# LTLA/batchelor

Hardware: AMD Instinct MI355X
Metric: cells/sec corrected (reducedMNN engine, 50 PCs) (higher is better)
Workload: dtype fp16 MFMA candidate pass (f32 accumulate) + FP64 exact re-rank; 1 GPU; config3: 8 synthetic Gaussian batches x 100000 cells x 50 PCs, k=20, merge.order=1..8, inputs resident in HBM; parallelism=single GPU, exact_fallback_queries=990

## Files before the change

batchelor_amd/csrc/abi.hip:

```cpp
#include <algorithm>
#include <chrono>
#include <climits>
#include <cstddef>
#include <cmath>
#include <cstdlib>
#include <cstring>
#include <functional>
#include <limits>
#include <memory>
#include <thread>
#include <vector>

#include "bmx_common.hpp"
#include "bmx_ops.hpp"
#include "engine.hpp"
#include "gene_var_host.hpp"
#include "host_xfer.hpp"
#include "mnn_correct.hpp"
#include "rccl_dyn.hpp"
#include "resident_batches.hpp"

struct bmx_engine {
    std::unique_ptr<bmx::Engine> impl;
};
// ... 141 lines not shown
        }
    });
}

void bmx_trim_caches(void) {
    bmx::DevBlockCache::release_global();
    bmx::StreamPool::release_all();
}

int64_t bmx_last_knn_exact_fallbacks(void) { return g_last_fallbacks; }

void bmx_set_force_exact_knn(int32_t on) { g_force_exact = on; }

int32_t bmx_dev_set(const char* name, int32_t value) {
    if (!name) return BMX_ERR_ARG;
    bmx::DevKnobs& k = bmx::dev_knobs();
    const std::string n(name);
    if (n == "knn_tier") k.knn_tier = value;
    else if (n == "sample") k.sample = value;
    else if (n == "split_c") k.split_c = value;
    else if (n == "force_c") k.force_c = value;
    else if (n == "no_margin") k.no_margin = value;
    else if (n == "asv_fast") k.asv_fast = value;
    else if (n == "asv_cap") k.asv_cap = value;
    else if (n == "sample_split") k.sample_split = value;
    else if (n == "lk_seed") k.lk_seed = value;
    else if (n == "asv_modes") k.asv_modes = value;
    else if (n == "asv_sync") k.asv_sync = value;
    else if (n == "tau_replay") k.tau_replay = value;
    else if (n == "exchange_always") k.exchange_always = value;
    else if (n == "refine_wave") k.refine_wave = value;
    else if (n == "asv_wide") k.asv_wide = value;
    else if (n == "asv_chunk") k.asv_chunk = value;
    else if (n == "reset") k = bmx::DevKnobs();
    else {
        g_last_error = "bmx_dev_set: unknown knob '" + n + "'";
        return BMX_ERR_ARG;
    }
    return BMX_OK;
}

int32_t bmx_dev_get(const char* name, int64_t* value) {
    if (!name || !value) return BMX_ERR_ARG;
    return guarded([&] {
        const std::string n(name);
        unsigned long long t[8];
        if (n == "asv_literal_cells" || n == "asv_fallback_cells" || n == "asv_tiled_cells") {
            bmx::asv_tally_read(t, false);
            *value = (int64_t)t[n == "asv_literal_cells" ? 0 : (n == "asv_fallback_cells" ? 1 : 2)];
        } else if (n == "asv_ticks_stream" || n == "asv_ticks_wait" || n == "asv_ticks_cells") {
            bmx::asv_ticks_read(t);
            *value = (int64_t)t[n == "asv_ticks_stream" ? 0 : (n == "asv_ticks_wait" ? 1 : 2)];
        } else if (n == "asv_ticks_literal" || n == "asv_ticks_chains" || n == "asv_literal_addends" || n == "asv_chain_tiles") {
            bmx::asv_ticks_read(t);
            *value = (int64_t)t[n == "asv_ticks_literal" ? 4 : (n == "asv_ticks_chains" ? 5 : (n == "asv_literal_addends" ? 6 : 7))];
        } else if (n == "delta_gene_tile" || n == "delta_pair_chunk") {
            *value = n == "delta_gene_tile" ? bmx::DELTA_GENE_TILE : bmx::DELTA_PAIR_CHUNK;
        } else if (n == "delta_sparse_gene_tile") {
            *value = bmx::DELTA_SPARSE_GENE_TILE;
        } else if (n == "genevar_gene_tile" || n == "genevar_chunk") {
            *value = n == "genevar_gene_tile" ? bmx::GENEVAR_GENE_TILE : bmx::GENEVAR_CHUNK;
        } else if (n == "cluster_sparse_gene_tile") {
            *value = bmx::CLUSTER_SPARSE_GENE_TILE;
        } else if (n == "pca_sparse_row_segment") {
            *value = bmx::PCA_SPARSE_ROW_SEGMENT;
        } else if (n == "asv_tally_reset") {
// ... 747 lines not shown
```

batchelor_amd/csrc/host_basics.hpp:

```cpp
#pragma once
#include <cstdint>
#include <stdexcept>
#include <string>

#include "../../include/batchelor_mi355x.h"

namespace bmx {

struct Error : std::runtime_error {
    int code;
    Error(int c, const std::string& m) : std::runtime_error(m), code(c) {}
};

struct DevKnobs {
    int knn_tier = 0;
    int sample = -1;
    int split_c = 0;
    int force_c = 0;
    int no_margin = 0;
    int asv_fast = 0;
    int asv_cap = -1;
    int asv_modes = 0;
    int asv_sync = 0;
    int tau_replay = 0;
    int lk_seed = 1;
    int sample_split = -1;
    int exchange_always = 0;
    int refine_wave = 0;
    int asv_wide = 0;
    int asv_chunk = 0;
};

inline int cdiv(int64_t a, int64_t b) { return (int)((a + b - 1) / b); }
inline int64_t round_up(int64_t a, int64_t b) { return (a + b - 1) / b * b; }

}
```

batchelor_amd/csrc/knn.hip:

```cpp
#include "knn_internal.hpp"

#include <algorithm>
#include <atomic>
#include <chrono>
#include <cmath>
#include <cstdio>
#include <thread>

namespace bmx {
namespace {

using namespace sel;

__global__ void colsum_partial(const double* __restrict__ X, const int32_t* __restrict__ rows, int n, int d,
                               int rows_per_block, int stride, double* __restrict__ partial) {
    __shared__ double sm[4][64];
    const int c0 = threadIdx.x & 63, rl = threadIdx.x >> 6;
    const int r0 = blockIdx.x * rows_per_block;
    const int r1 = min(n, r0 + rows_per_block);
    for (int cb = 0; cb < d; cb += 64) {
        const int c = cb + c0;
        double s = 0.0;
        if (c < d)
            for (int r = r0 + rl; r < r1; r += 4) {
// ... 83 lines not shown
        pe.eps_qr = 6.0;
        pe.eps_split = 1.5 * 3.03 * 2.0 * 1.52587890625e-05;
        pe.eps_den = 0.0;
        pe.scaled = 0;
    }
    return pe;
}

}

int candidate_tiers(int d, int k, int nr, Tier out[2]) {
    const int only = dev_knobs().knn_tier;
    int n = 0;
    if (k > 36) return 0;
    const int KS1 = k <= 20 ? BMX_KS1 : 48, KS2 = k <= 20 ? 24 : 40;
    const int ns1 = f16_pick_ns(d, KS1);
    if (ns1 && nr > 2 * KS1 && (only == 0 || only == 1)) out[n++] = Tier{1, ns1, KS1};
    const int ns2 = bf16_pick_ns(d);
    if (ns2 && !(KS2 == 40 && ns2 > 16) && nr > 2 * KS2 && (only == 0 || only == 2)) out[n++] = Tier{2, ns2, KS2};
    return n;
}

namespace {

void candidate_pass(hipStream_t stream, KnnWorkspace& ws, const Tier& T, const double* X, const int32_t* ref_rows, int nr,
                    const double* Qs, const int32_t* qrs, int nq, int d, int k, int32_t* io, double* dout,
                    int32_t* flagged, double* flag_bound, const float* seed_d2, const double* centre, double* kth_out) {
    const int NS = T.NS, KS = T.KS;
    ws.last_variant = T.id == 1 ? 3 : 2;
    const PassPlan plan = plan_candidate_pass(T.id, NS, KS, T.id == 1 ? 256 : 32 * bf16_ncons(NS, KS),
                                              T.id == 1 ? f16_rows_per_slot(NS, KS) : 32, nq, nr, seed_d2 != nullptr, dev_knobs());
    const int nq_pad = plan.nq_pad, nqb = plan.nqb, S = plan.S, C = plan.C, chunk_len = plan.chunk_len, nr_pad = plan.nr_pad;
    const int nchunks = C;
    if (debug_prints())
        fprintf(stderr, "[bmx] knn tier %d: nq=%d nr=%d d=%d NS=%d KS=%d S=%d C=%d chunk=%d full-range blocks=%d of %d\n", T.id,
                nq, nr, d, NS, KS, S, C, chunk_len, C > 1 ? plan.n_full : nqb, nqb);

    const int KPw = 8 * NS;
    float* pq = ws.pq.reserve((size_t)nq_pad * KPw);
    float* pr = ws.pr.reserve((size_t)(nr_pad + 256) * KPw);
    double* qn2 = ws.qn2.reserve(nq_pad);
    double* rn2 = ws.rn2.reserve(nr_pad);
    double* mean = ws.mean.reserve((size_t)d + 2);
    unsigned long long* maxbits = reinterpret_cast<unsigned long long*>(mean + d);
    int32_t* cand = ws.cand.reserve((size_t)nq_pad * nchunks * KS);
    float* cand_v = ws.cand_v.reserve((size_t)nq_pad * nchunks * KS);
    float* tau = ws.tau.reserve((size_t)nq_pad * nchunks);
    uint32_t* tau_g = ws.tau_g.reserve(nq_pad);
    unsigned long long* slots = ws.maxslots.reserve(64 * 16);

    if (!centre) {
        const int cstride = std::max(1, nr / 16384);
        const int ncs = cdiv(nr, cstride);
        const int rpb = 256;
        const int nb = cdiv(ncs, rpb);
        double* red = ws.red.reserve((size_t)nb * d);
        hipLaunchKernelGGL(colsum_partial, dim3(nb), dim3(256), 0, stream, X, ref_rows, ncs, d, rpb, cstride, red);
        BMX_LAUNCH_CHECK();
        hipLaunchKernelGGL(colsum_final, dim3(cdiv(d, 64)), dim3(64), 0, stream, red, nb, d, 1.0 / ncs, mean);
        BMX_LAUNCH_CHECK();
        centre = mean;
    }
    const PassEps pe = tier_pass_eps(T, d);
    PassLaunch L{reinterpret_cast<const uint16_t*>(pq), reinterpret_cast<const uint16_t*>(pr), nqb, 0, plan.sample_range_len,
                 plan.sample_nranges, S, 0, nchunks, tau_g, 1, cand, cand_v, tau};
    const bool no_margin = dev_knobs().no_margin != 0;
    auto go = [&](const PassLaunch& l) {
        return T.id == 1 ? f16_launch(stream, ws, NS, KS, l) : bf16_launch(stream, ws, NS, KS, l);
    };
    bool ok = true;
    unsigned long long* zero_slots = nullptr;
    if (T.id == 1) {
        if (!ws.slots_clean) BMX_HIP(hipMemsetAsync(slots, 0, 64 * 16 * sizeof(unsigned long long), stream));
        float* margin = no_margin ? nullptr : ws.margin.reserve(nq_pad);
        uint32_t* tau_seed = seed_d2 ? ws.tau_seed.reserve(nq_pad) : nullptr;
        f16_prep_all(stream, X, ref_rows, nr, nr_pad, Qs, qrs, nq, nq_pad, d, NS, centre, reinterpret_cast<uint16_t*>(pr),
                     reinterpret_cast<uint16_t*>(pq), rn2, qn2, maxbits, slots, flagged, margin, pe, seed_d2, tau_seed,
                     S == 0 || plan.CS > 1 ? tau_g : nullptr);
        if (margin) {
            L.margin = margin;
            L.k = k;
        }
        L.tau_seed = tau_seed;
        zero_slots = slots;
        ws.slots_clean = false;
        if (S > 0) {
            float* lists = nullptr;
            if (L.nranges > 1 && margin) {
                lists = ws.samp_lists.reserve((size_t)nq_pad * L.nranges * KS);
                L.cand_v = lists;
            }
            ok = go(L);
            if (lists) f16_sample_merge(stream, lists, L.nranges, KS, nq, k, margin, tau_g);
            L.cand_v = cand_v;
        }
    } else {
        ws.slots_clean = false;
        BMX_HIP(hipMemsetAsync(maxbits, 0, sizeof(unsigned long long), stream));
        bf16_prep(stream, X, ref_rows, nr, nr_pad, d, NS, centre, 0, reinterpret_cast<uint16_t*>(pr), rn2, maxbits, slots);
        bf16_prep(stream, Qs, qrs, nq, nq_pad, d, NS, centre, 1, reinterpret_cast<uint16_t*>(pq), qn2, maxbits, slots);
        if (S == 0) {
            hipLaunchKernelGGL(fill_u32, dim3(cdiv(nq_pad, 256)), dim3(256), 0, stream, tau_g, nq_pad, 0xFF800000u);
            BMX_LAUNCH_CHECK();
        }
        if (S > 0) ok = go(L);
        if (seed_d2) {
            hipLaunchKernelGGL(seed_tau_kernel, dim3(cdiv(nq_pad, 256)), dim3(256), 0, stream, seed_d2, qn2, maxbits, nq, nq_pad,
                               pe, tau_g);
            BMX_LAUNCH_CHECK();
        }
        BMX_HIP(hipMemsetAsync(flagged, 0, sizeof(int32_t), stream));
    }
    L.first_begin = 0;
    L.range_len = chunk_len;
    L.nranges = C;
    L.n_full = C > 1 ? plan.n_full : 0;
    L.r_limit = nr_pad;
    L.sample = 0;
    const int replay = T.id == 1 ? dev_knobs().tau_replay : 0;
    if (replay == 2 && ws.replay_idx < ws.tau_rec.size() && ws.tau_rec[ws.replay_idx].cap >= (size_t)nq_pad) {
        hipLaunchKernelGGL(tau_apply_kernel, dim3(cdiv(nq_pad, 256)), dim3(256), 0, stream,
                           (const uint32_t*)ws.tau_rec[ws.replay_idx].p, nq_pad, tau_g);
        BMX_LAUNCH_CHECK();
    }
    ok = ok && go(L);
    if (replay == 1) {
        if (ws.tau_rec.size() <= ws.replay_idx) ws.tau_rec.resize(ws.replay_idx + 1);
        hipLaunchKernelGGL(tau_record_kernel, dim3(cdiv(nq_pad, 256)), dim3(256), 0, stream, (const float*)tau, nchunks, nq_pad,
                           ws.tau_rec[ws.replay_idx].reserve((size_t)nq_pad));
        BMX_LAUNCH_CHECK();
    }
    if (replay) ++ws.replay_idx;
    if (!ok) throw Error(BMX_ERR_ARG, "kNN: unsupported padded dimension");
    refine_launch(stream, ws, plan, KS, pe, PassLists{cand, cand_v, tau, qn2, maxbits}, X, ref_rows, Qs, qrs, nq, d, k, seed_d2,
                  io, dout, flagged, flag_bound, zero_slots, kth_out);
    if (zero_slots) ws.slots_clean = true;
    if (debug_prints()) {
        std::vector<int32_t> hc((size_t)nq * nchunks * KS);
        BMX_HIP(hipMemcpyAsync(hc.data(), cand, hc.size() * sizeof(int32_t), hipMemcpyDeviceToHost, stream));
        ws.sync(stream);
        size_t valid = 0;
        for (int32_t v : hc) valid += v >= 0;
        fprintf(stderr, "[bmx] candidates per query after the top-k pass: %.1f (of %d slots)\n", (double)valid / nq,
                nchunks * KS);
    }
// ... 109 lines not shown
```

batchelor_amd/csrc/knn_f16.hip:

```cpp
#include "knn_internal.hpp"

#include <cmath>
#include <string>

namespace bmx {
namespace {

using namespace sel;
typedef _Float16 f16x8 __attribute__((ext_vector_type(8)));

constexpr int NCONS = 8;
constexpr int NPROD = 2;
#ifndef BMX_NSERV
#define BMX_NSERV 4
#endif
__host__ __device__ constexpr int serv_waves(int NS) { return NS <= 5 ? BMX_NSERV : 2; }
constexpr int NQ = NCONS * 32;
constexpr int QCAP = 64;
#ifndef BMX_DRAIN_MIN
#define BMX_DRAIN_MIN 16
#endif
#ifndef BMX_SPRIO
#define BMX_SPRIO 0
#endif
#ifndef BMX_CPRIO_LO
#define BMX_CPRIO_LO 0
#endif
#ifndef BMX_CPRIO_HI
#define BMX_CPRIO_HI 1
#endif
#ifndef BMX_HEAD
#define BMX_HEAD 4
#endif
#ifndef BMX_RING_MAX
#define BMX_RING_MAX 4
#endif
#ifndef BMX_NPIV
#define BMX_NPIV 4
#endif
#ifndef BMX_PSLEEP
#define BMX_PSLEEP 1
#endif
constexpr int EPI_CONS = 20;
constexpr int DRAIN_MIN = BMX_DRAIN_MIN;
constexpr int HEAD = BMX_HEAD;

__device__ __forceinline__ uint16_t f32_to_f16_bits(float f) {
    const _Float16 h = (_Float16)f;
    return __builtin_bit_cast(uint16_t, h);
}
__device__ __forceinline__ float f16_bits_to_f32(uint16_t b) { return (float)__builtin_bit_cast(_Float16, b); }

__host__ __device__ __forceinline__ double f16_scale(double max_n2) {
    const double rm = sqrt(max_n2);
    if (!(rm > 1e-150) || !(rm < 1e150)) return 1.0;
    int e = 0;
    (void)frexp(48.0 / rm, &e);
    return ldexp(1.0, e - 1);
}

template <int PHASE>
__device__ __forceinline__ double prep_rows(char* smem_pp, int block, const double* __restrict__ X,
                                            const int32_t* __restrict__ rows, int n, int d, int NS,
                                            const double* __restrict__ mean, int is_query, uint16_t* __restrict__ P,
                                            double* __restrict__ n2, unsigned long long* __restrict__ max_slots,
                                            double scale) {
    const int K = 16 * NS;
    float* xs = reinterpret_cast<float*>(smem_pp);
// ... 125 lines not shown
        double m = __longlong_as_double((long long)slots[(size_t)threadIdx.x * 16]);
        for (int o = 1; o < 64; o <<= 1) m = fmax(m, __shfl_xor(m, o));
        if (threadIdx.x == 0) {
            sh_max = m;
            if (blockIdx.x == 0) {
                *max_n2_bits = (unsigned long long)__double_as_longlong(m);
                if (flagged0) *flagged0 = 0;
            }
        }
    }
    __syncthreads();
    const double max_rn2 = sh_max;
    const double scale = f16_scale(max_rn2);
    if ((int)blockIdx.x < nrb) {
        (void)prep_rows<1>(smem_pp, blockIdx.x, X, rrows, nr, d, NS, mean, 0, Pr, rn2, nullptr, scale);
        return;
    }
    const int qb = blockIdx.x - nrb;
    const double s = prep_rows<1>(smem_pp, qb, Q, qrows, nq, d, NS, mean, 1, Pq, qn2, nullptr, scale);
    const int rr = threadIdx.x >> 3, sub = threadIdx.x & 7;
    if (sub == 0) {
        const int q = qb * 32 + rr;
        const bool live = q < nq;
        const double nn = live ? qn2[q] : 0.0;
        (void)s;
        if (margin) margin[q] = live ? pass_margin(nn, max_rn2, pe) : 0.f;
        uint32_t ts = 0xFF800000u;
        if (seed_d2) ts = live ? pass_seed_tau((double)seed_d2[q], nn, max_rn2, pe) : f32_orderable(-__builtin_inff());
        if (tau_seed) tau_seed[q] = ts;
        if (tau_init) tau_init[q] = ts;
    }
}

__host__ __device__ constexpr int lds_fixed_bytes() { return NCONS * QCAP * 20 + NQ * 4 + NQ * 4 + NQ * 4 + 512; }
__host__ __device__ constexpr int ring_slots_for(int NS, int LCAP, int TP) {
    const int rest = 160 * 1024 - lds_fixed_bytes() - NQ * LCAP * 8;
    const int n = rest / (TP * 2 * NS * 1024);
    return n > BMX_RING_MAX ? BMX_RING_MAX : n;
}
#ifndef BMX_LCAP_MAX
#define BMX_LCAP_MAX 56
#endif
#ifndef BMX_TP_MAX
#define BMX_TP_MAX 2
#endif
__host__ __device__ constexpr int tile_pairs_for(int NS, int KS) {
    return (BMX_TP_MAX >= 2 && KS + 16 <= BMX_LCAP_MAX && ring_slots_for(NS, KS + 16, 2) >= 3) ? 2 : 1;
}
__host__ __device__ constexpr int list_cap(int NS, int KS) {
    const int TP = tile_pairs_for(NS, KS);
    for (int c = BMX_LCAP_MAX; c >= KS + 16; c -= 8)
        if (ring_slots_for(NS, c, TP) >= (TP == 2 ? 3 : 2)) return c;
    return KS + 16 <= 64 ? KS + 16 : 64;
}

__device__ __forceinline__ int lds_load_volatile(const int* p) {
    return __hip_atomic_load(p, __ATOMIC_RELAXED, __HIP_MEMORY_SCOPE_WORKGROUP);
}
__device__ __forceinline__ int mbcnt64(unsigned long long m) {
    return __builtin_amdgcn_mbcnt_hi((uint32_t)(m >> 32), __builtin_amdgcn_mbcnt_lo((uint32_t)m, 0u));
}

#ifdef BMX_STAMPS
__device__ unsigned long long bmx_dbg16[48];
#define STAMP() __builtin_readcyclecounter()
#endif

template <int NS, int KS, int LCAP, bool SAMPLE>
__global__ __launch_bounds__((NCONS + NPROD + serv_waves(NS)) * 64) void knn_topk_f16(
    const uint16_t* __restrict__ Pq, const uint16_t* __restrict__ PrF, int first_begin, int range_len, int r_limit,
    int n_full, int nranges, int out_chunk0, int out_nchunks, uint32_t* __restrict__ tau_g, int32_t* __restrict__ cand,
    float* __restrict__ cand_v, float* __restrict__ tau_out, const float* __restrict__ margin_g, int kq,
    const uint32_t* __restrict__ tau_seed) {
    constexpr int TILE_BYTES = NS * 1024;
    constexpr int TP = tile_pairs_for(NS, KS);
    constexpr int SLOT_BYTES = TP * 2 * TILE_BYTES;
    constexpr int NSLOT = ring_slots_for(NS, LCAP, TP);
    static_assert(NSLOT >= 2, "LDS ring");
    static_assert(LCAP <= 64 && LCAP > KS, "one list entry per lane during compaction");
    constexpr int KEEP_MAX = KS + 11 < LCAP - 4 ? KS + 11 : LCAP - 4;
    static_assert(KEEP_MAX >= KS, "list capacity");
    constexpr int NSERV = serv_waves(NS);
    static_assert(NCONS % NSERV == 0 && (NCONS / NSERV) % 2 == 0, "a service wave's consumers: whole groups of 64 queries");
    static_assert((QCAP & (QCAP - 1)) == 0 && QCAP >= 64, "queue positions wrap by masking; one group can hold 64 records");

    extern __shared__ __attribute__((aligned(16))) char smem[];
    char* ring = smem;
    unsigned long long* lists = reinterpret_cast<unsigned long long*>(smem + NSLOT * SLOT_BYTES);
    float* qvals = reinterpret_cast<float*>(lists + NQ * LCAP);
    uint32_t* qtags = reinterpret_cast<uint32_t*>(qvals + NCONS * QCAP * 4);
    int* cnt = reinterpret_cast<int*>(qtags + NCONS * QCAP);
    float* tauL = reinterpret_cast<float*>(cnt + NQ);
    float* mgL = tauL + NQ;
    int* ready = reinterpret_cast<int*>(mgL + NQ);
    int* done = ready + NSLOT;
    int* wrL = done + NSLOT;
    int* rdL = wrL + NCONS;
    int* stL = rdL + NCONS;
#ifdef BMX_EXP_ROWFILTER
    float* rtau = reinterpret_cast<float*>(stL + NCONS);
    if (threadIdx.x < 32) rtau[threadIdx.x] = -__builtin_inff();
#endif

    const int tid = threadIdx.x, lane = tid & 63;
    const int wave = __builtin_amdgcn_readfirstlane(tid >> 6);
    int qblock = blockIdx.x, rng = 0, nrng = 1, r_begin = first_begin, r_end = r_limit;
    if ((int)blockIdx.x >= n_full) {
        const int nsplit = (gridDim.x - n_full) / nranges, jx = blockIdx.x - n_full;
        rng = jx / nsplit;
        qblock = n_full + (jx - rng * nsplit);
        nrng = nranges;
        r_begin = first_begin + rng * range_len;
        r_end = min(r_limit, r_begin + range_len);
    }
    const int ntiles = (r_end - r_begin) >> 5;
    const int nslots = ntiles / (2 * TP);
    const int out_chunk = out_chunk0 + rng;
    if (tid < 2 * NSLOT + 3 * NCONS) ready[tid] = 0;
    if (tid < NQ) {
        cnt[tid] = 0;
        tauL[tid] = (!SAMPLE && tau_g) ? orderable_f32(tau_g[qblock * NQ + tid]) : __builtin_inff();
        mgL[tid] = (!SAMPLE && margin_g) ? margin_g[qblock * NQ + tid] : 0.f;
    }
    __syncthreads();
    const bool shared_tau = !SAMPLE && tau_g != nullptr && nrng > 1;

#ifdef BMX_STAMPS
    unsigned long long dbg_ncomp = 0, dbg_comp = 0, dbg_rounds = 0;
#endif
    auto compact = [&](const int c, const int jj, const bool exact) __attribute__((always_inline)) {
        unsigned long long* mylists = lists + c * 32 * LCAP;
        int* mycnt = cnt + c * 32;
        const int n_raw = __builtin_amdgcn_readfirstlane(lds_load_volatile(&mycnt[jj]));
        const int n = n_raw < LCAP ? n_raw : LCAP;
        if (n <= KS && (n < kq || margin_g == nullptr)) return;
#ifdef BMX_STAMPS
        const unsigned long long c0 = STAMP();
        ++dbg_ncomp;
#endif
        const unsigned long long raw = lane < n ? mylists[jj * LCAP + lane] : 0ull;
        const uint32_t key =
            lane < n ? (((f32_orderable(__uint_as_float((uint32_t)(raw >> 32))) >> 1) & ~63u) | (uint32_t)lane)
                     : 0x7FFFFFFFu;
        unsigned long long M = 0, keep = 0;
        int pl = 0, kept = 0x7FFFFFFF, nkeep = 0;
        uint32_t pk = 0;
        float newtau = 0.f;
        bool cut_done = false;
        auto select_rank = [&](unsigned long long B, const int target) __attribute__((always_inline)) {
            int it = 0;
            for (;;) {
                const int rot = (it * 29 + jj * 7) & 63;
// ... 495 lines not shown
                    for (int u = 0; u < 4; ++u) {
                        unsigned long long mu = __builtin_amdgcn_ballot_w64(g[u] < tau);
                        if (mu == 0) continue;
                        const int c = __builtin_popcountll(mu);
                        if (wr + c - rd_seen > QCAP) {
                            wait_room(c);
                            const float tl =
                                __hip_atomic_load(&tauL[wave * 32 + j], __ATOMIC_RELAXED, __HIP_MEMORY_SCOPE_WORKGROUP);
                            tau = tl < tau ? tl : tau;
                            mu = __builtin_amdgcn_ballot_w64(g[u] < tau);
                        }
                        if (mu) {
                            spill(u, mu);
                            __atomic_signal_fence(__ATOMIC_SEQ_CST);
                            lane0_store(&wrL[wave], wr);
                        }
                    }
#ifdef BMX_STAMPS
                    dbg_evc += STAMP() - dbg_e0;
#endif
                    return mn;
                }
                wait_room(tot);
            }
#pragma unroll
            for (int u = 0; u < 4; ++u) spill(u, m[u]);
#ifdef BMX_STAMPS
            dbg_evc += STAMP() - dbg_e0;
#endif
            return mn;
        }
    };

    if (wave >= NCONS / 2)
        __builtin_amdgcn_s_setprio(BMX_CPRIO_HI);
    else
        __builtin_amdgcn_s_setprio(BMX_CPRIO_LO);
    __builtin_amdgcn_s_waitcnt(0x0F70);
    if (nslots > 0) {
        typedef __attribute__((address_space(3))) const char* lds_cptr;
        typedef __attribute__((address_space(3))) const f32x4* lds_f4ptr;
        lds_cptr ring_lane = (lds_cptr)ring + lane * 16;
        asm volatile("" : "+v"(ring_lane));
        spin_until_staged(0, 0);
        __atomic_signal_fence(__ATOMIC_SEQ_CST);
        {
            const lds_f4ptr tp = (lds_f4ptr)ring_lane;
#pragma unroll
            for (int s = 0; s < NS; ++s) {
                a[s] = tp[s * 64];
                b[s] = tp[(NS + s) * 64];
            }
        }
        if constexpr (TP == 1) hand_back(0);
        poll(1 % NSLOT);
        auto tile_pair = [&](const lds_f4ptr tp, const int t0, const int hand_back_pos) __attribute__((always_inline)) {
            f32x16 accA, accB;
#ifdef BMX_EXP_ROWFILTER
            if constexpr (!SAMPLE) {
#ifdef BMX_EXP_ROWFILTER_NOLDS
#pragma unroll
                for (int u = 0; u < 4; ++u) {
                    rt[u] = f32x4{rt0, rt0, rt0, rt0};
                    asm volatile("" : "+v"(rt[u]));
                }
#else
// ... 19 lines not shown
                __builtin_amdgcn_sched_group_barrier(0x008, 1, 0);
                __builtin_amdgcn_sched_group_barrier(0x100, 1, 0);
            }
            __builtin_amdgcn_sched_barrier(0);
            if (hand_back_pos >= 0) hand_back(hand_back_pos);
            const float mnA = sift(accA, t0);
            const float mnB = sift(accB, t0 + 1);
            if constexpr (SAMPLE) {
                sample_insert(fminf(fminf(mnA, mnB), mnB));
            }
        };
        for (int sl0 = 0; sl0 < nslots; sl0 += NSLOT) {
#pragma unroll
            for (int k = 0; k < NSLOT; ++k) {
                const int sl = sl0 + k;
                if (sl >= nslots) break;
                const int kn = (k + 1) % NSLOT;
                if constexpr (TP == 2) {
                    __builtin_amdgcn_s_waitcnt(0xC07F);
                    tile_pair((lds_f4ptr)(ring_lane + k * SLOT_BYTES + 2 * TILE_BYTES), 4 * sl, k);
                }
                __builtin_amdgcn_s_waitcnt(0xC07F);
                if constexpr (!SAMPLE) asm("v_min_f32 %0, %0, %1" : "+v"(tau) : "v"(tau_next));
                spin_until_staged(sl + 1, kn);
                __atomic_signal_fence(__ATOMIC_SEQ_CST);
                poll((kn + 1) % NSLOT);
                tile_pair((lds_f4ptr)(ring_lane + kn * SLOT_BYTES), 2 * TP * sl + 2 * (TP - 1), TP == 1 ? kn : -1);
            }
        }
    }
    __builtin_amdgcn_s_setprio(0);

    if constexpr (SAMPLE) {
        const uint32_t mine = f32_orderable(best[KS / 2 - 1]), other = __shfl_xor(mine, 32);
        uint32_t start = max(mine, other);
        if constexpr (KS / 2 <= 24) {
            if (margin_g && kq >= 1 && kq <= KS) {
                float part[KS / 2];
#pragma unroll
                for (int e = 0; e < KS / 2; ++e) part[e] = __shfl_xor(best[e], 32);
                float uk = __builtin_inff();
#pragma unroll
                for (int i = 0; i < KS / 2; ++i) {
                    int r = i;
#pragma unroll
                    for (int e = 0; e < KS / 2; ++e) r += (part[e] < best[i] || (part[e] == best[i] && h == 1)) ? 1 : 0;
                    uk = r == kq - 1 ? best[i] : uk;
                }
                uk = fminf(uk, __shfl_xor(uk, 32));
                const float tm = uk + margin_g[q] + fabsf(uk) * 2.384185791015625e-07f;
                if (tm == tm) start = min(start, f32_orderable(tm));
            }
        }
        if (h == 0) {
            if (nrng > 1) atomicMin(&tau_g[q], start);
            else tau_g[q] = tau_seed ? min(start, tau_seed[q]) : start;
        }
        if (nrng > 1 && cand_v) {
            float* dst = cand_v + ((int64_t)q * nrng + rng) * KS + h * (KS / 2);
#pragma unroll
            for (int e = 0; e < KS / 2; e += 4)
                *reinterpret_cast<f32x4*>(dst + e) = f32x4{best[e], best[e + 1], best[e + 2], best[e + 3]};
        }
#ifdef BMX_STAMPS
        if (lane == 0) {
            atomicAdd(&bmx_dbg16[0], STAMP() - dbg_t0);
            atomicAdd(&bmx_dbg16[1], dbg_spin);
            atomicAdd(&bmx_dbg16[8], (unsigned long long)ntiles);
            atomicAdd(&bmx_dbg16[9], 1ull);
        }
#endif
    } else {
        __atomic_signal_fence(__ATOMIC_SEQ_CST);
        lane0_store(&wrL[wave], wr);
        lane0_store(&stL[wave], 2);
        while (__builtin_amdgcn_readfirstlane(lds_load_volatile(&stL[wave])) != 3) __builtin_amdgcn_s_sleep(2);
        __atomic_signal_fence(__ATOMIC_SEQ_CST);
        out_lists(wave, 0, EPI_CONS);
#ifdef BMX_STAMPS
        if (lane == 0) {
            atomicAdd(&bmx_dbg16[0], STAMP() - dbg_t0);
            atomicAdd(&bmx_dbg16[1], dbg_spin);
            atomicAdd(&bmx_dbg16[6], dbg_evt);
            atomicAdd(&bmx_dbg16[7], dbg_grp);
            atomicAdd(&bmx_dbg16[8], (unsigned long long)ntiles);
            atomicAdd(&bmx_dbg16[9], 1ull);
            atomicAdd(&bmx_dbg16[10], dbg_evc);
            atomicAdd(&bmx_dbg16[12], dbg_qwait);
        }
#endif
    }
}

template <int NS, int KS>
void launch(hipStream_t stream, KnnWorkspace& ws, const PassLaunch& L) {
    constexpr int LCAP = list_cap(NS, KS);
    constexpr int TP = tile_pairs_for(NS, KS);
    constexpr size_t lds =
        (size_t)ring_slots_for(NS, LCAP, TP) * TP * 2 * NS * 1024 + (size_t)NQ * LCAP * 8 + lds_fixed_bytes();
    static_assert(lds <= 160 * 1024, "LDS budget");
    ensure_dynamic_lds(reinterpret_cast<const void*>(&knn_topk_f16<NS, KS, LCAP, false>), lds);
    ensure_dynamic_lds(reinterpret_cast<const void*>(&knn_topk_f16<NS, KS, LCAP, true>), lds);
    std::pair<hipEvent_t, hipEvent_t> ev{nullptr, nullptr};
    if (ws.profile) {
        ev = ws.next_events(L.sample ? 0 : 1);
        BMX_HIP(hipEventRecord(ev.first, stream));
    }
    if (!L.sample)
        ws.last_kernel = "knn_topk_f16<" + std::to_string(NS) + ", " + std::to_string(KS) + ", " + std::to_string(LCAP) +
                         ", false>";
    const int items = L.n_full + (L.nqb - L.n_full) * L.nranges;
    if (L.sample)
        hipLaunchKernelGGL((knn_topk_f16<NS, KS, LCAP, true>), dim3(items), dim3((NCONS + NPROD + serv_waves(NS)) * 64), lds, stream,
                           L.pq, L.pr, L.first_begin, L.range_len, L.r_limit, L.n_full, L.nranges, L.out_chunk0,
                           L.out_nchunks, L.tau_g, L.cand, L.cand_v, L.tau, L.margin, L.k, L.tau_seed);
    else
        hipLaunchKernelGGL((knn_topk_f16<NS, KS, LCAP, false>), dim3(items), dim3((NCONS + NPROD + serv_waves(NS)) * 64), lds, stream,
                           L.pq, L.pr, L.first_begin, L.range_len, L.r_limit, L.n_full, L.nranges, L.out_chunk0,
                           L.out_nchunks, L.tau_g, L.cand, L.cand_v, L.tau, L.margin, L.k, (const uint32_t*)nullptr);
    BMX_LAUNCH_CHECK();
    if (ws.profile) BMX_HIP(hipEventRecord(ev.second, stream));
#ifdef BMX_STAMPS
    {
        if (L.sample) fprintf(stderr, "(sample pass) ");
        unsigned long long hh[48];
        BMX_HIP(hipStreamSynchronize(stream));
        BMX_HIP(hipMemcpyFromSymbol(hh, HIP_SYMBOL(bmx_dbg16), sizeof(hh)));
        const double nt = (double)hh[8];
        const double sw = hh[14] ? (double)hh[14] : 1.0;
        fprintf(stderr,
                "[stamps f16] consumers=%.0f tiles/wave=%.0f cyc/tile=%.0f spin/tile=%.0f evpath/tile=%.0f qwait/tile=%.0f "
                "event tiles=%.3f groups/tile=%.3f | service waves=%.0f cyc=%.0f drain=%.0f (%.0f passes, %.0f cyc each) "
                "compact=%.0f (%.0f calls, %.1f rounds each) idle polls=%.0f\n",
                (double)hh[9], nt / hh[9], hh[0] / nt, hh[1] / nt, hh[10] / nt, hh[12] / nt, hh[6] / nt, hh[7] / nt,
                (double)hh[14], hh[13] / sw, hh[2] / sw, hh[3] / sw, hh[3] ? (double)hh[2] / hh[3] : 0.0, hh[5] / sw,
                hh[4] / sw, hh[4] ? (double)hh[11] / hh[4] : 0.0, hh[15] / sw);
        unsigned long long z[48] = {0};
        BMX_HIP(hipMemcpyToSymbol(HIP_SYMBOL(bmx_dbg16), z, sizeof(z)));
    }
#endif
}

}

namespace {
// ... 50 lines not shown
    hipLaunchKernelGGL(knn_prep_f16_rq, dim3(nr_pad / 32 + nq_pad / 32), dim3(256), lds, stream, X, rrows, nr, nr_pad / 32, Q, qrows,
                       nq, d, NS, mean, Pr, Pq, rn2, qn2, (const unsigned long long*)slots, maxbits, flagged0, margin, pe, seed_d2,
                       tau_seed, tau_init);
    BMX_LAUNCH_CHECK();
}

bool f16_launch(hipStream_t stream, KnnWorkspace& ws, int NS, int KS, const PassLaunch& L) {
#define BMX_CASE(N)                       \
    case N:                               \
        if (KS == BMX_KS1)                \
            launch<N, BMX_KS1>(stream, ws, L); \
        else if constexpr (N <= 4)        \
            launch<N, 48>(stream, ws, L); \
        else                              \
            return false;                 \
        return true;
    switch (NS) {
        BMX_CASE(1)
        BMX_CASE(2)
        BMX_CASE(3)
        BMX_CASE(4)
        BMX_CASE(5)
        BMX_CASE(6)
        BMX_CASE(7)
        BMX_CASE(8)
        default:
            return false;
    }
#undef BMX_CASE
}

double f16_scale_host(double max_n2) { return f16_scale(max_n2); }
int f16_rows_per_slot(int NS, int KS) { return 64 * tile_pairs_for(NS, KS); }

}
```

batchelor_amd/csrc/knn_internal.hpp:

```cpp
#pragma once
#include "bmx_common.hpp"
#include "knn_plan.hpp"
#include "knn_select.hpp"

namespace bmx {

struct PassLaunch {
    const uint16_t* pq;
    const uint16_t* pr;
    int nqb, first_begin, range_len, nranges, r_limit, out_chunk0, out_nchunks;
    uint32_t* tau_g;
    int sample;
    int32_t* cand;
    float* cand_v;
    float* tau;
    int n_full = 0;
    const float* margin = nullptr;
    int k = 0;
    const uint32_t* tau_seed = nullptr;
};
int bf16_pick_ns(int d);
int bf16_ncons(int NS, int KS);
void bf16_prep(hipStream_t stream, const double* X, const int32_t* rows, int n, int n_pad, int d, int NS,
               const double* mean, int is_query, uint16_t* P, double* n2, unsigned long long* maxbits,
               unsigned long long* slots);
bool bf16_launch(hipStream_t stream, KnnWorkspace& ws, int NS, int KS, const PassLaunch& L);
int f16_pick_ns(int d, int KS);
int f16_rows_per_slot(int NS, int KS);
void f16_prep_all(hipStream_t stream, const double* X, const int32_t* rrows, int nr, int nr_pad, const double* Q,
                  const int32_t* qrows, int nq, int nq_pad, int d, int NS, const double* mean, uint16_t* Pr, uint16_t* Pq,
                  double* rn2, double* qn2, unsigned long long* maxbits, unsigned long long* slots, int32_t* flagged0,
                  float* margin, const sel::PassEps& pe, const float* seed_d2, uint32_t* tau_seed, uint32_t* tau_init);
bool f16_launch(hipStream_t stream, KnnWorkspace& ws, int NS, int KS, const PassLaunch& L);
void f16_sample_merge(hipStream_t stream, const float* lists, int nranges, int KS, int nq, int k, const float* margin,
                      uint32_t* tau_g);

struct Tier {
    int id;
    int NS, KS;
};
int candidate_tiers(int d, int k, int nr, Tier out[2]);
void search_tiers(hipStream_t stream, KnnWorkspace& ws, const Tier* tiers, int ntiers, int t, const double* X,
                  const int32_t* ref_rows, int nr, const double* Qs, const int32_t* qrs, int nq, int d, int k, int32_t* io,
                  double* dout, const float* seed_d2 = nullptr, const double* centre = nullptr, double* kth_out = nullptr);
int read_count(hipStream_t stream, KnnWorkspace& ws, const int32_t* dev);

struct PassLists {
    const int32_t* cand;
    const float* cand_v;
    const float* tau;
    const double* qn2;
    const unsigned long long* maxbits;
};
void refine_launch(hipStream_t stream, KnnWorkspace& ws, const PassPlan& plan, int KS, const sel::PassEps& pe,
                   const PassLists& lists, const double* X, const int32_t* ref_rows, const double* Qs, const int32_t* qrs,
                   int nq, int d, int k, const float* seed_d2, int32_t* io, double* dout, int32_t* flagged,
                   double* flag_bound, unsigned long long* zero_slots, double* kth_out);

int32_t* launch_bounded_sweep(hipStream_t stream, KnnWorkspace& ws, const double* X, const int32_t* ref_rows, int nr,
                              const double* Qs, const int32_t* qrs, int d, int k, int32_t* io, double* dout,
                              const int32_t* list, const double* bounds, int count, int dev_cap, bool seeded, int32_t* opt);
// ... 13 lines not shown
```

Measured before the change: 9.417 million cells/s.

## Add 64-query-per-wave consumers for the f16 sample pass

Adds a sample-pass kernel variant for the NS=4, KS=32 instance in which each consumer wave handles 64 queries: it issues two MFMAs per loaded reference fragment, keeps per-lane minima directly in registers, and drops the service waves and LDS candidate lists. This raises reuse of each staged reference tile and removes queue and service overhead in the sampling stage. The sample launch is replanned with a doubled query block, so the query-side buffers are padded to the larger size. Because the fragment-min insertion differs from the service-wave path, the sampled thresholds may be looser, which could increase work in later passes. The new path is on by default through a knob.

```diff
diff --git a/batchelor_amd/csrc/abi.hip b/batchelor_amd/csrc/abi.hip
--- a/batchelor_amd/csrc/abi.hip
+++ b/batchelor_amd/csrc/abi.hip
@@ -197,6 +197,7 @@
     else if (n == "refine_wave") k.refine_wave = value;
     else if (n == "asv_wide") k.asv_wide = value;
     else if (n == "asv_chunk") k.asv_chunk = value;
+    else if (n == "wide_consumers") k.wide_consumers = value;
     else if (n == "reset") k = bmx::DevKnobs();
     else {
         g_last_error = "bmx_dev_set: unknown knob '" + n + "'";
diff --git a/batchelor_amd/csrc/host_basics.hpp b/batchelor_amd/csrc/host_basics.hpp
--- a/batchelor_amd/csrc/host_basics.hpp
+++ b/batchelor_amd/csrc/host_basics.hpp
@@ -29,6 +29,7 @@
     int refine_wave = 0;
     int asv_wide = 0;
     int asv_chunk = 0;
+    int wide_consumers = 1;
 };
 
 inline int cdiv(int64_t a, int64_t b) { return (int)((a + b - 1) / b); }
diff --git a/batchelor_amd/csrc/knn.hip b/batchelor_amd/csrc/knn.hip
--- a/batchelor_amd/csrc/knn.hip
+++ b/batchelor_amd/csrc/knn.hip
@@ -139,21 +139,26 @@
                                               T.id == 1 ? f16_rows_per_slot(NS, KS) : 32, nq, nr, seed_d2 != nullptr, dev_knobs());
     const int nq_pad = plan.nq_pad, nqb = plan.nqb, S = plan.S, C = plan.C, chunk_len = plan.chunk_len, nr_pad = plan.nr_pad;
     const int nchunks = C;
+    const int unit_s = T.id == 1 ? f16_queries_per_block(NS, KS, true, dev_knobs().wide_consumers != 0) : plan.unit;
+    const PassPlan splan = unit_s == plan.unit ? plan
+                                               : plan_candidate_pass(T.id, NS, KS, unit_s, f16_rows_per_slot(NS, KS), nq, nr,
+                                                                     seed_d2 != nullptr, dev_knobs());
+    const int nq_prep = std::max(nq_pad, splan.nq_pad);
     if (debug_prints())
         fprintf(stderr, "[bmx] knn tier %d: nq=%d nr=%d d=%d NS=%d KS=%d S=%d C=%d chunk=%d full-range blocks=%d of %d\n", T.id,
                 nq, nr, d, NS, KS, S, C, chunk_len, C > 1 ? plan.n_full : nqb, nqb);
 
     const int KPw = 8 * NS;
-    float* pq = ws.pq.reserve((size_t)nq_pad * KPw);
+    float* pq = ws.pq.reserve((size_t)nq_prep * KPw);
     float* pr = ws.pr.reserve((size_t)(nr_pad + 256) * KPw);
-    double* qn2 = ws.qn2.reserve(nq_pad);
+    double* qn2 = ws.qn2.reserve(nq_prep);
     double* rn2 = ws.rn2.reserve(nr_pad);
     double* mean = ws.mean.reserve((size_t)d + 2);
     unsigned long long* maxbits = reinterpret_cast<unsigned long long*>(mean + d);
     int32_t* cand = ws.cand.reserve((size_t)nq_pad * nchunks * KS);
     float* cand_v = ws.cand_v.reserve((size_t)nq_pad * nchunks * KS);
     float* tau = ws.tau.reserve((size_t)nq_pad * nchunks);
-    uint32_t* tau_g = ws.tau_g.reserve(nq_pad);
+    uint32_t* tau_g = ws.tau_g.reserve(nq_prep);
     unsigned long long* slots = ws.maxslots.reserve(64 * 16);
 
     if (!centre) {
@@ -169,8 +174,9 @@
         centre = mean;
     }
     const PassEps pe = tier_pass_eps(T, d);
-    PassLaunch L{reinterpret_cast<const uint16_t*>(pq), reinterpret_cast<const uint16_t*>(pr), nqb, 0, plan.sample_range_len,
-                 plan.sample_nranges, S, 0, nchunks, tau_g, 1, cand, cand_v, tau};
+    PassLaunch L{reinterpret_cast<const uint16_t*>(pq), reinterpret_cast<const uint16_t*>(pr), splan.nqb, 0, splan.sample_range_len,
+                 splan.sample_nranges, S, 0, nchunks, tau_g, 1, cand, cand_v, tau};
+    L.cw = unit_s == plan.unit ? 32 : 64;
     const bool no_margin = dev_knobs().no_margin != 0;
     auto go = [&](const PassLaunch& l) {
         return T.id == 1 ? f16_launch(stream, ws, NS, KS, l) : bf16_launch(stream, ws, NS, KS, l);
@@ -179,11 +185,11 @@
     unsigned long long* zero_slots = nullptr;
     if (T.id == 1) {
         if (!ws.slots_clean) BMX_HIP(hipMemsetAsync(slots, 0, 64 * 16 * sizeof(unsigned long long), stream));
-        float* margin = no_margin ? nullptr : ws.margin.reserve(nq_pad);
-        uint32_t* tau_seed = seed_d2 ? ws.tau_seed.reserve(nq_pad) : nullptr;
-        f16_prep_all(stream, X, ref_rows, nr, nr_pad, Qs, qrs, nq, nq_pad, d, NS, centre, reinterpret_cast<uint16_t*>(pr),
+        float* margin = no_margin ? nullptr : ws.margin.reserve(nq_prep);
+        uint32_t* tau_seed = seed_d2 ? ws.tau_seed.reserve(nq_prep) : nullptr;
+        f16_prep_all(stream, X, ref_rows, nr, nr_pad, Qs, qrs, nq, nq_prep, d, NS, centre, reinterpret_cast<uint16_t*>(pr),
                      reinterpret_cast<uint16_t*>(pq), rn2, qn2, maxbits, slots, flagged, margin, pe, seed_d2, tau_seed,
-                     S == 0 || plan.CS > 1 ? tau_g : nullptr);
+                     S == 0 || splan.CS > 1 ? tau_g : nullptr);
         if (margin) {
             L.margin = margin;
             L.k = k;
@@ -194,7 +200,7 @@
         if (S > 0) {
             float* lists = nullptr;
             if (L.nranges > 1 && margin) {
-                lists = ws.samp_lists.reserve((size_t)nq_pad * L.nranges * KS);
+                lists = ws.samp_lists.reserve((size_t)nq_prep * L.nranges * KS);
                 L.cand_v = lists;
             }
             ok = go(L);
@@ -218,6 +224,8 @@
         }
         BMX_HIP(hipMemsetAsync(flagged, 0, sizeof(int32_t), stream));
     }
+    L.nqb = nqb;
+    L.cw = 32;
     L.first_begin = 0;
     L.range_len = chunk_len;
     L.nranges = C;
diff --git a/batchelor_amd/csrc/knn_f16.hip b/batchelor_amd/csrc/knn_f16.hip
--- a/batchelor_amd/csrc/knn_f16.hip
+++ b/batchelor_amd/csrc/knn_f16.hip
@@ -1,3 +1,4 @@
+#include "knn_f16_budget.hpp"
 #include "knn_internal.hpp"
 
 #include <cmath>
@@ -7,16 +8,9 @@
 namespace {
 
 using namespace sel;
+using namespace f16cfg;
 typedef _Float16 f16x8 __attribute__((ext_vector_type(8)));
 
-constexpr int NCONS = 8;
-constexpr int NPROD = 2;
-#ifndef BMX_NSERV
-#define BMX_NSERV 4
-#endif
-__host__ __device__ constexpr int serv_waves(int NS) { return NS <= 5 ? BMX_NSERV : 2; }
-constexpr int NQ = NCONS * 32;
-constexpr int QCAP = 64;
 #ifndef BMX_DRAIN_MIN
 #define BMX_DRAIN_MIN 16
 #endif
@@ -31,9 +25,6 @@
 #endif
 #ifndef BMX_HEAD
 #define BMX_HEAD 4
-#endif
-#ifndef BMX_RING_MAX
-#define BMX_RING_MAX 4
 #endif
 #ifndef BMX_NPIV
 #define BMX_NPIV 4
@@ -225,27 +216,6 @@
     }
 }
 
-__host__ __device__ constexpr int lds_fixed_bytes() { return NCONS * QCAP * 20 + NQ * 4 + NQ * 4 + NQ * 4 + 512; }
-__host__ __device__ constexpr int ring_slots_for(int NS, int LCAP, int TP) {
-    const int rest = 160 * 1024 - lds_fixed_bytes() - NQ * LCAP * 8;
-    const int n = rest / (TP * 2 * NS * 1024);
-    return n > BMX_RING_MAX ? BMX_RING_MAX : n;
-}
-#ifndef BMX_LCAP_MAX
-#define BMX_LCAP_MAX 56
-#endif
-#ifndef BMX_TP_MAX
-#define BMX_TP_MAX 2
-#endif
-__host__ __device__ constexpr int tile_pairs_for(int NS, int KS) {
-    return (BMX_TP_MAX >= 2 && KS + 16 <= BMX_LCAP_MAX && ring_slots_for(NS, KS + 16, 2) >= 3) ? 2 : 1;
-}
-__host__ __device__ constexpr int list_cap(int NS, int KS) {
-    const int TP = tile_pairs_for(NS, KS);
-    for (int c = BMX_LCAP_MAX; c >= KS + 16; c -= 8)
-        if (ring_slots_for(NS, c, TP) >= (TP == 2 ? 3 : 2)) return c;
-    return KS + 16 <= 64 ? KS + 16 : 64;
-}
 
 __device__ __forceinline__ int lds_load_volatile(const int* p) {
     return __hip_atomic_load(p, __ATOMIC_RELAXED, __HIP_MEMORY_SCOPE_WORKGROUP);
@@ -259,8 +229,44 @@
 #define STAMP() __builtin_readcyclecounter()
 #endif
 
-template <int NS, int KS, int LCAP, bool SAMPLE>
-__global__ __launch_bounds__((NCONS + NPROD + serv_waves(NS)) * 64) void knn_topk_f16(
+template <int KS>
+__device__ __forceinline__ void sample_finish(const float (&bst)[KS / 2], const int qq, const int h, const int nrng, const int rng,
+                                              const int kq, const float* __restrict__ margin_g, uint32_t* __restrict__ tau_g,
+                                              const uint32_t* __restrict__ tau_seed, float* __restrict__ cand_v) {
+    const uint32_t mine = f32_orderable(bst[KS / 2 - 1]), other = __shfl_xor(mine, 32);
+    uint32_t start = max(mine, other);
+    if constexpr (KS / 2 <= 24) {
+        if (margin_g && kq >= 1 && kq <= KS) {
+            float part[KS / 2];
+#pragma unroll
+            for (int e = 0; e < KS / 2; ++e) part[e] = __shfl_xor(bst[e], 32);
+            float uk = __builtin_inff();
+#pragma unroll
+            for (int i = 0; i < KS / 2; ++i) {
+                int r = i;
+#pragma unroll
+                for (int e = 0; e < KS / 2; ++e) r += (part[e] < bst[i] || (part[e] == bst[i] && h == 1)) ? 1 : 0;
+                uk = r == kq - 1 ? bst[i] : uk;
+            }
+            uk = fminf(uk, __shfl_xor(uk, 32));
+            const float tm = uk + margin_g[qq] + fabsf(uk) * 2.384185791015625e-07f;
+            if (tm == tm) start = min(start, f32_orderable(tm));
+        }
+    }
+    if (h == 0) {
+        if (nrng > 1) atomicMin(&tau_g[qq], start);
+        else tau_g[qq] = tau_seed ? min(start, tau_seed[qq]) : start;
+    }
+    if (nrng > 1 && cand_v) {
+        float* dst = cand_v + ((int64_t)qq * nrng + rng) * KS + h * (KS / 2);
+#pragma unroll
+        for (int e = 0; e < KS / 2; e += 4)
+            *reinterpret_cast<f32x4*>(dst + e) = f32x4{bst[e], bst[e + 1], bst[e + 2], bst[e + 3]};
+    }
+}
+
+template <int NS, int KS, int LCAP, bool SAMPLE, int CW = 32>
+__global__ __launch_bounds__(pass_waves(NS, SAMPLE, CW) * 64) void knn_topk_f16(
     const uint16_t* __restrict__ Pq, const uint16_t* __restrict__ PrF, int first_begin, int range_len, int r_limit,
     int n_full, int nranges, int out_chunk0, int out_nchunks, uint32_t* __restrict__ tau_g, int32_t* __restrict__ cand,
     float* __restrict__ cand_v, float* __restrict__ tau_out, const float* __restrict__ margin_g, int kq,
@@ -277,15 +283,18 @@
     static_assert(NCONS % NSERV == 0 && (NCONS / NSERV) % 2 == 0, "a service wave's consumers: whole groups of 64 queries");
     static_assert((QCAP & (QCAP - 1)) == 0 && QCAP >= 64, "queue positions wrap by masking; one group can hold 64 records");
 
+    static_assert(CW == 32 || (CW == 64 && SAMPLE && wide_sample_instance(NS, KS)), "64-query consumers: that sample pass only");
+    constexpr int NQ = NCONS * CW;
+    constexpr int LQ = CW == 32 ? NQ : 0;
     extern __shared__ __attribute__((aligned(16))) char smem[];
     char* ring = smem;
     unsigned long long* lists = reinterpret_cast<unsigned long long*>(smem + NSLOT * SLOT_BYTES);
-    float* qvals = reinterpret_cast<float*>(lists + NQ * LCAP);
+    float* qvals = reinterpret_cast<float*>(lists + LQ * LCAP);
     uint32_t* qtags = reinterpret_cast<uint32_t*>(qvals + NCONS * QCAP * 4);
     int* cnt = reinterpret_cast<int*>(qtags + NCONS * QCAP);
-    float* tauL = reinterpret_cast<float*>(cnt + NQ);
-    float* mgL = tauL + NQ;
-    int* ready = reinterpret_cast<int*>(mgL + NQ);
+    float* tauL = reinterpret_cast<float*>(cnt + LQ);
+    float* mgL = tauL + LQ;
+    int* ready = reinterpret_cast<int*>(mgL + LQ);
     int* done = ready + NSLOT;
     int* wrL = done + NSLOT;
     int* rdL = wrL + NCONS;
@@ -310,7 +319,7 @@
     const int nslots = ntiles / (2 * TP);
     const int out_chunk = out_chunk0 + rng;
     if (tid < 2 * NSLOT + 3 * NCONS) ready[tid] = 0;
-    if (tid < NQ) {
+    if (tid < LQ) {
         cnt[tid] = 0;
         tauL[tid] = (!SAMPLE && tau_g) ? orderable_f32(tau_g[qblock * NQ + tid]) : __builtin_inff();
         mgL[tid] = (!SAMPLE && margin_g) ? margin_g[qblock * NQ + tid] : 0.f;
@@ -872,6 +881,111 @@
         }
     };
 
+    if constexpr (CW == 64) {
+        static_assert(TP == 2, "64-query consumers: slots of four tiles");
+        const int qa = qblock * NQ + wave * 64 + j;
+        f16x8 qf[2][NS];
+        {
+            const f32x4* src = reinterpret_cast<const f32x4*>(Pq + (int64_t)qa * (16 * NS) + h * (8 * NS));
+#pragma unroll
+            for (int s = 0; s < NS; ++s) {
+                qf[0][s] = __builtin_bit_cast(f16x8, src[s]);
+                qf[1][s] = __builtin_bit_cast(f16x8, src[32 * 2 * NS + s]);
+            }
+        }
+        float bw[2][KS / 2];
+#pragma unroll
+        for (int i = 0; i < KS / 2; ++i) bw[0][i] = bw[1][i] = __builtin_inff();
+        auto insert = [&](float(&bst)[KS / 2], const float x) __attribute__((always_inline)) {
+#pragma unroll
+            for (int i = KS / 2 - 1; i > 0; --i) bst[i] = __builtin_amdgcn_fmed3f(bst[i - 1], bst[i], x);
+            bst[0] = fminf(fminf(bst[0], x), x);
+        };
+        float pinf = __builtin_inff();
+        asm volatile("" : "+v"(pinf));
+        auto lane_min = [&](const f32x16& acc, const float third) __attribute__((always_inline)) {
+            float t[5];
+#pragma unroll
+            for (int u = 0; u < 5; ++u) {
+                t[u] = fminf(fminf(acc[3 * u], acc[3 * u + 1]), acc[3 * u + 2]);
+                asm("" : "+v"(t[u]));
+            }
+            float u0 = fminf(fminf(t[0], t[1]), t[2]), u1 = fminf(fminf(t[3], t[4]), acc[15]);
+            asm("" : "+v"(u0), "+v"(u1));
+            return fminf(fminf(u0, u1), third);
+        };
+        if (wave >= NCONS / 2)
+            __builtin_amdgcn_s_setprio(BMX_CPRIO_HI);
+        else
+            __builtin_amdgcn_s_setprio(BMX_CPRIO_LO);
+        __builtin_amdgcn_s_waitcnt(0x0F70);
+        if (nslots > 0) {
+            typedef __attribute__((address_space(3))) const char* lds_cptr;
+            typedef __attribute__((address_space(3))) const f32x4* lds_f4ptr;
+            lds_cptr ring_lane = (lds_cptr)ring + lane * 16;
+            asm volatile("" : "+v"(ring_lane));
+            f32x4 fr[NS];
+            spin_until_staged(0, 0);
+            __atomic_signal_fence(__ATOMIC_SEQ_CST);
+#pragma unroll
+            for (int s = 0; s < NS; ++s) fr[s] = ((lds_f4ptr)ring_lane)[s * 64];
+            poll(1 % NSLOT);
+            float even0 = pinf, even1 = pinf;
+            auto tile = [&](const lds_f4ptr nx, const bool odd, const int hand_back_pos) __attribute__((always_inline)) {
+                f32x16 acc0, acc1;
+#pragma unroll
+                for (int e = 0; e < 16; ++e) acc0[e] = acc1[e] = 0.f;
+                __builtin_amdgcn_sched_barrier(0);
+#pragma unroll
+                for (int s = 0; s < NS; ++s) {
+                    const f16x8 f = __builtin_bit_cast(f16x8, fr[s]);
+                    acc0 = __builtin_amdgcn_mfma_f32_32x32x16_f16(f, qf[0][s], acc0, 0, 0, 0);
+                    acc1 = __builtin_amdgcn_mfma_f32_32x32x16_f16(f, qf[1][s], acc1, 0, 0, 0);
+                    fr[s] = nx[s * 64];
+                }
+#pragma unroll
+                for (int s = 0; s < NS; ++s) {
+                    __builtin_amdgcn_sched_group_barrier(0x008, 2, 0);
+                    __builtin_amdgcn_sched_group_barrier(0x100, 1, 0);
+                }
+                __builtin_amdgcn_sched_barrier(0);
+                if (hand_back_pos >= 0) hand_back(hand_back_pos);
+                float m0 = lane_min(acc0, odd ? even0 : pinf), m1 = lane_min(acc1, odd ? even1 : pinf);
+                asm volatile("" : "+v"(m0), "+v"(m1));
+                if (odd) {
+                    insert(bw[0], m0);
+                    insert(bw[1], m1);
+                } else {
+                    even0 = m0;
+                    even1 = m1;
+                }
+            };
+            for (int sl0 = 0; sl0 < nslots; sl0 += NSLOT) {
+#pragma unroll
+                for (int k = 0; k < NSLOT; ++k) {
+                    const int sl = sl0 + k;
+                    if (sl >= nslots) break;
+                    const int kn = (k + 1) % NSLOT;
+                    const lds_cptr slot = ring_lane + k * SLOT_BYTES;
+                    __builtin_amdgcn_s_waitcnt(0xC07F);
+                    tile((lds_f4ptr)(slot + TILE_BYTES), false, -1);
+                    __builtin_amdgcn_s_waitcnt(0xC07F);
+                    tile((lds_f4ptr)(slot + 2 * TILE_BYTES), true, -1);
+                    __builtin_amdgcn_s_waitcnt(0xC07F);
+                    tile((lds_f4ptr)(slot + 3 * TILE_BYTES), false, k);
+                    __builtin_amdgcn_s_waitcnt(0xC07F);
+                    spin_until_staged(sl + 1, kn);
+                    __atomic_signal_fence(__ATOMIC_SEQ_CST);
+                    poll((kn + 1) % NSLOT);
+                    tile((lds_f4ptr)(ring_lane + kn * SLOT_BYTES), true, -1);
+                }
+            }
+        }
+        __builtin_amdgcn_s_setprio(0);
+        sample_finish<KS>(bw[0], qa, h, nrng, rng, kq, margin_g, tau_g, tau_seed, cand_v);
+        sample_finish<KS>(bw[1], qa + 32, h, nrng, rng, kq, margin_g, tau_g, tau_seed, cand_v);
+        return;
+    }
     if (wave >= NCONS / 2)
         __builtin_amdgcn_s_setprio(BMX_CPRIO_HI);
     else
@@ -957,36 +1071,7 @@
     __builtin_amdgcn_s_setprio(0);
 
     if constexpr (SAMPLE) {
-        const uint32_t mine = f32_orderable(best[KS / 2 - 1]), other = __shfl_xor(mine, 32);
-        uint32_t start = max(mine, other);
-        if constexpr (KS / 2 <= 24) {
-            if (margin_g && kq >= 1 && kq <= KS) {
-                float part[KS / 2];
-#pragma unroll
-                for (int e = 0; e < KS / 2; ++e) part[e] = __shfl_xor(best[e], 32);
-                float uk = __builtin_inff();
-#pragma unroll
-                for (int i = 0; i < KS / 2; ++i) {
-                    int r = i;
-#pragma unroll
-                    for (int e = 0; e < KS / 2; ++e) r += (part[e] < best[i] || (part[e] == best[i] && h == 1)) ? 1 : 0;
-                    uk = r == kq - 1 ? best[i] : uk;
-                }
-                uk = fminf(uk, __shfl_xor(uk, 32));
-                const float tm = uk + margin_g[q] + fabsf(uk) * 2.384185791015625e-07f;
-                if (tm == tm) start = min(start, f32_orderable(tm));
-            }
-        }
-        if (h == 0) {
-            if (nrng > 1) atomicMin(&tau_g[q], start);
-            else tau_g[q] = tau_seed ? min(start, tau_seed[q]) : start;
-        }
-        if (nrng > 1 && cand_v) {
-            float* dst = cand_v + ((int64_t)q * nrng + rng) * KS + h * (KS / 2);
-#pragma unroll
-            for (int e = 0; e < KS / 2; e += 4)
-                *reinterpret_cast<f32x4*>(dst + e) = f32x4{best[e], best[e + 1], best[e + 2], best[e + 3]};
-        }
+        sample_finish<KS>(best, q, h, nrng, rng, kq, margin_g, tau_g, tau_seed, cand_v);
 #ifdef BMX_STAMPS
         if (lane == 0) {
             atomicAdd(&bmx_dbg16[0], STAMP() - dbg_t0);
@@ -1020,9 +1105,7 @@
 template <int NS, int KS>
 void launch(hipStream_t stream, KnnWorkspace& ws, const PassLaunch& L) {
     constexpr int LCAP = list_cap(NS, KS);
-    constexpr int TP = tile_pairs_for(NS, KS);
-    constexpr size_t lds =
-        (size_t)ring_slots_for(NS, LCAP, TP) * TP * 2 * NS * 1024 + (size_t)NQ * LCAP * 8 + lds_fixed_bytes();
+    constexpr size_t lds = pass_lds_bytes(NS, KS);
     static_assert(lds <= 160 * 1024, "LDS budget");
     ensure_dynamic_lds(reinterpret_cast<const void*>(&knn_topk_f16<NS, KS, LCAP, false>), lds);
     ensure_dynamic_lds(reinterpret_cast<const void*>(&knn_topk_f16<NS, KS, LCAP, true>), lds);
@@ -1035,7 +1118,16 @@
         ws.last_kernel = "knn_topk_f16<" + std::to_string(NS) + ", " + std::to_string(KS) + ", " + std::to_string(LCAP) +
                          ", false>";
     const int items = L.n_full + (L.nqb - L.n_full) * L.nranges;
-    if (L.sample)
+    if (L.sample && L.cw == 64) {
+        if constexpr (wide_sample_instance(NS, KS)) {
+            ensure_dynamic_lds(reinterpret_cast<const void*>(&knn_topk_f16<NS, KS, LCAP, true, 64>), lds);
+            hipLaunchKernelGGL((knn_topk_f16<NS, KS, LCAP, true, 64>), dim3(items), dim3(pass_waves(NS, true, 64) * 64), lds, stream,
+                               L.pq, L.pr, L.first_begin, L.range_len, L.r_limit, L.n_full, L.nranges, L.out_chunk0,
+                               L.out_nchunks, L.tau_g, L.cand, L.cand_v, L.tau, L.margin, L.k, L.tau_seed);
+        } else {
+            throw Error(BMX_ERR_ARG, "kNN: no 64-query sample pass for this instance");
+        }
+    } else if (L.sample)
         hipLaunchKernelGGL((knn_topk_f16<NS, KS, LCAP, true>), dim3(items), dim3((NCONS + NPROD + serv_waves(NS)) * 64), lds, stream,
                            L.pq, L.pr, L.first_begin, L.range_len, L.r_limit, L.n_full, L.nranges, L.out_chunk0,
                            L.out_nchunks, L.tau_g, L.cand, L.cand_v, L.tau, L.margin, L.k, L.tau_seed);
@@ -1152,5 +1244,8 @@
 
 double f16_scale_host(double max_n2) { return f16_scale(max_n2); }
 int f16_rows_per_slot(int NS, int KS) { return 64 * tile_pairs_for(NS, KS); }
-
-}
+int f16_queries_per_block(int NS, int KS, bool sample, bool wide) {
+    return queries_per_block(NS, KS, sample, wide);
+}
+
+}
diff --git a/batchelor_amd/csrc/knn_f16_budget.hpp b/batchelor_amd/csrc/knn_f16_budget.hpp
--- /dev/null
+++ b/batchelor_amd/csrc/knn_f16_budget.hpp
@@ -0,0 +1,59 @@
+#pragma once
+
+#if defined(__HIPCC__)
+#define BMX_F16_HD __host__ __device__
+#else
+#define BMX_F16_HD
+#endif
+
+namespace bmx {
+namespace f16cfg {
+
+constexpr int NCONS = 8;
+constexpr int NPROD = 2;
+#ifndef BMX_NSERV
+#define BMX_NSERV 4
+#endif
+BMX_F16_HD constexpr int serv_waves(int NS) { return NS <= 5 ? BMX_NSERV : 2; }
+constexpr int NQ = NCONS * 32;
+constexpr int QCAP = 64;
+#ifndef BMX_RING_MAX
+#define BMX_RING_MAX 4
+#endif
+
+BMX_F16_HD constexpr int lds_fixed_bytes() { return NCONS * QCAP * 20 + NQ * 4 + NQ * 4 + NQ * 4 + 512; }
+BMX_F16_HD constexpr int ring_slots_for(int NS, int LCAP, int TP) {
+    const int rest = 160 * 1024 - lds_fixed_bytes() - NQ * LCAP * 8;
+    const int n = rest / (TP * 2 * NS * 1024);
+    return n > BMX_RING_MAX ? BMX_RING_MAX : n;
+}
+#ifndef BMX_LCAP_MAX
+#define BMX_LCAP_MAX 56
+#endif
+#ifndef BMX_TP_MAX
+#define BMX_TP_MAX 2
+#endif
+BMX_F16_HD constexpr int tile_pairs_for(int NS, int KS) {
+    return (BMX_TP_MAX >= 2 && KS + 16 <= BMX_LCAP_MAX && ring_slots_for(NS, KS + 16, 2) >= 3) ? 2 : 1;
+}
+BMX_F16_HD constexpr int list_cap(int NS, int KS) {
+    const int TP = tile_pairs_for(NS, KS);
+    for (int c = BMX_LCAP_MAX; c >= KS + 16; c -= 8)
+        if (ring_slots_for(NS, c, TP) >= (TP == 2 ? 3 : 2)) return c;
+    return KS + 16 <= 64 ? KS + 16 : 64;
+}
+BMX_F16_HD constexpr int pass_lds_bytes(int NS, int KS) {
+    const int LCAP = list_cap(NS, KS), TP = tile_pairs_for(NS, KS);
+    return ring_slots_for(NS, LCAP, TP) * TP * 2 * NS * 1024 + NQ * LCAP * 8 + lds_fixed_bytes();
+}
+
+BMX_F16_HD constexpr bool wide_sample_instance(int NS, int KS) { return NS == 4 && KS == 32; }
+BMX_F16_HD constexpr int pass_waves(int NS, bool SAMPLE, int CW) {
+    return NCONS + NPROD + (SAMPLE && CW == 64 ? 0 : serv_waves(NS));
+}
+BMX_F16_HD constexpr int queries_per_block(int NS, int KS, bool sample, bool wide) {
+    return NCONS * (sample && wide && wide_sample_instance(NS, KS) ? 64 : 32);
+}
+
+}
+}
diff --git a/batchelor_amd/csrc/knn_internal.hpp b/batchelor_amd/csrc/knn_internal.hpp
--- a/batchelor_amd/csrc/knn_internal.hpp
+++ b/batchelor_amd/csrc/knn_internal.hpp
@@ -18,6 +18,7 @@
     const float* margin = nullptr;
     int k = 0;
     const uint32_t* tau_seed = nullptr;
+    int cw = 32;
 };
 int bf16_pick_ns(int d);
 int bf16_ncons(int NS, int KS);
@@ -27,6 +28,7 @@
 bool bf16_launch(hipStream_t stream, KnnWorkspace& ws, int NS, int KS, const PassLaunch& L);
 int f16_pick_ns(int d, int KS);
 int f16_rows_per_slot(int NS, int KS);
+int f16_queries_per_block(int NS, int KS, bool sample, bool wide);
 void f16_prep_all(hipStream_t stream, const double* X, const int32_t* rrows, int nr, int nr_pad, const double* Q,
                   const int32_t* qrows, int nq, int nq_pad, int d, int NS, const double* mean, uint16_t* Pr, uint16_t* Pq,
                   double* rn2, double* qn2, unsigned long long* maxbits, unsigned long long* slots, int32_t* flagged0,
```

Result: no change. 9.407 million cells/s (-0.1%).
